# syghmon/bridges-with-reinforcement-learning

Measured on AMD Instinct MI355X. Metric: env-steps/sec (vectorised assembly_gym, tower_height=4), higher is better.
Workload: dtype f64

## Files before the change

### bridges-with-reinforcement-learning_amd/csrc/api.hip

```cpp
#include <hip/hip_runtime.h>
#include <cstdio>
#include <cstdlib>
#include <cstring>
#include <new>

#include "env_kernels.hip"
#include "ops_kernels.hip"
#include "dqn_kernels.hip"
#include "mlp_kernels.hip"
#include "conv_kernels.hip"
#include "conv_train_kernels.hip"

using namespace bridges;

static thread_local char g_err[512] = "";

static int fail_hip(hipError_t e, const char* what) {
    snprintf(g_err, sizeof(g_err), "%s: %s", what, hipGetErrorString(e));
    return BRIDGES_E_HIP;
}
static int fail_arg(const char* what) {
    snprintf(g_err, sizeof(g_err), "bad argument: %s", what);
    return BRIDGES_E_ARG;
}
// ... 172 lines not shown
    *out = env;
    return BRIDGES_OK;
}

static void free_events(bridges_env* env) {
    for (int i = 0; i < env->ev_cap; ++i) {
        (void)hipEventDestroy(env->ev_start[i]);
        (void)hipEventDestroy(env->ev_stop[i]);
    }
    delete[] env->ev_start;
    delete[] env->ev_stop;
    env->ev_start = env->ev_stop = nullptr;
    env->ev_cap = env->ev_used = 0;
}

int bridges_env_destroy(bridges_env* env) {
    if (!env) return BRIDGES_OK;
    free_events(env);
    if (env->raster_done) (void)hipEventDestroy(env->raster_done);
    (void)hipFree(env->tt_dev);
    (void)hipHostFree(env->h_total);
    delete env;
    return BRIDGES_OK;
}

int bridges_gate_create(bridges_gate** out) {
    if (!out) return fail_arg("gate_create");
    bridges_gate* g = new (std::nothrow) bridges_gate();
    if (!g) return fail_arg("oom");
    g->last = nullptr;
    *out = g;
    return BRIDGES_OK;
}

int bridges_gate_destroy(bridges_gate* gate) {
    delete gate;
    return BRIDGES_OK;
}

int bridges_env_set_gate(bridges_env* env, bridges_gate* gate) {
    if (!env) return fail_arg("set_gate");
    if (gate && !env->raster_done) HIP_TRY(hipEventCreateWithFlags(&env->raster_done, hipEventDisableTiming));
    env->gate = gate;
    return BRIDGES_OK;
}

int bridges_env_timing_begin(bridges_env* env, int32_t max_launches) {
    if (!env || max_launches <= 0 || max_launches > (1 << 16)) return fail_arg("timing_begin");
    free_events(env);
    env->ev_start = new (std::nothrow) hipEvent_t[max_launches];
    env->ev_stop = new (std::nothrow) hipEvent_t[max_launches];
    if (!env->ev_start || !env->ev_stop) {
        delete[] env->ev_start;
        delete[] env->ev_stop;
        env->ev_start = env->ev_stop = nullptr;
        return fail_arg("oom");
    }
    for (int i = 0; i < max_launches; ++i) {
        HIP_TRY(hipEventCreate(&env->ev_start[i]));
        HIP_TRY(hipEventCreate(&env->ev_stop[i]));
        env->ev_cap = i + 1;
    }
    env->ev_used = 0;
    return BRIDGES_OK;
}

int bridges_env_timing_end(bridges_env* env, double* raster_ms_total, int32_t* n_launches) {
    if (!env || !raster_ms_total || !n_launches) return fail_arg("timing_end");
    double total = 0.0;
    for (int i = 0; i < env->ev_used; ++i) {
        HIP_TRY(hipEventSynchronize(env->ev_stop[i]));
        float ms = 0.f;
        HIP_TRY(hipEventElapsedTime(&ms, env->ev_start[i], env->ev_stop[i]));
        total += ms;
    }
    *raster_ms_total = total;
    *n_launches = env->ev_used;
    free_events(env);
    return BRIDGES_OK;
}

static int refresh(bridges_env* env, hipStream_t s, int after_step) {
    const DevCtx& c = env->ctx;
    if (int rc = launch("k_scan", k_scan, dim3(1), dim3(SCAN_THREADS), 0, s, c, after_step)) return rc;
    if (int rc = launch("k_enumerate", k_enumerate, dim3(c.E), dim3(WAVE), 0, s, c)) return rc;
    const long long items_est = candidate_estimate(env) + c.E;
    long long rblocks = ceil_div(items_est, 4);
    if (rblocks > env->max_blocks) rblocks = env->max_blocks;
    const bool timed = env->ev_cap > 0 && env->ev_used < env->ev_cap;
    if (env->gate && env->gate->last) HIP_TRY(hipStreamWaitEvent(s, env->gate->last, 0));
    if (timed) HIP_TRY(hipEventRecord(env->ev_start[env->ev_used], s));
    if (!env->has_tasks) {
        if (int rc = launch("k_raster", env->max_faces <= 4 ? k_raster<4> : k_raster<MAXV>, dim3((unsigned)rblocks), dim3(256), 0, s, c))
            return rc;
    } else if (env->tasks.n_obstacles == 0) {
        if (int rc = launch("k_raster (per-env tables)", env->max_faces <= 4 ? k_raster<4, true> : k_raster<MAXV, true>,
                            dim3((unsigned)rblocks), dim3(256), 0, s, c))
            return rc;
    } else if (int rc = launch("k_raster (per-env tables and obstacles)", env->max_faces <= 4 ? k_raster<4, true, const uint64_t*> : k_raster<MAXV, true, const uint64_t*>,
                               dim3((unsigned)rblocks), dim3(256), 0, s, c, (const uint64_t*)env->tasks.env_obstacle_bits)) {
        return rc;
    }
    if (timed) { HIP_TRY(hipEventRecord(env->ev_stop[env->ev_used], s)); env->ev_used++; }
    if (env->gate) {
        HIP_TRY(hipEventRecord(env->raster_done, s));
        env->gate->last = env->raster_done;
    }
    return launch("k_select", k_select, dim3(c.E), dim3(WAVE), 0, s, c, 0);
}

static int task_features(bridges_env* env, void* stream, int mode) {
    if (env->family.family != BRIDGES_FAMILY_NONE && env->family_thr)
        return launch("k_task_features (weighted task family)", k_task_features<bridges_task_family, const uint64_t*>, dim3(env->ctx.E),
                      dim3(TASK_THREADS), 0, stream, env->ctx, env->tasks, mode, env->family, env->family_thr);
    if (env->family.family != BRIDGES_FAMILY_NONE)
        return launch("k_task_features (task family)", k_task_features<bridges_task_family>, dim3(env->ctx.E), dim3(TASK_THREADS), 0,
                      stream, env->ctx, env->tasks, mode, env->family);
    return launch("k_task_features", k_task_features<>, dim3(env->ctx.E), dim3(TASK_THREADS), 0, stream, env->ctx, env->tasks, mode);
}

int bridges_env_reset(bridges_env* env, void* stream) {
    if (!env) return fail_arg("null env");
    if (int rc = launch("k_reset", k_reset, dim3(env->ctx.E), dim3(WAVE), 0, stream, env->ctx)) return rc;
    if (env->has_tasks)
        if (int rc = task_features(env, stream, TASK_RESET)) return rc;
    return refresh(env, (hipStream_t)stream, 0);
}

int bridges_env_step(bridges_env* env, void* stream) {
    if (!env) return fail_arg("null env");
    if (!env->has_tasks) {
        if (int rc = launch("k_step", k_step<>, dim3(env->ctx.E), dim3(WAVE), 0, stream, env->ctx)) return rc;
    } else {
        if (int rc = launch("k_step (per-env targets)", k_step<const double*>, dim3(env->ctx.E), dim3(WAVE), 0, stream, env->ctx,
                            (const double*)env->tasks.env_targets))
            return rc;
        if (env->tasks.sample || env->tasks.sample_obstacles || env->family.family != BRIDGES_FAMILY_NONE)
            if (int rc = task_features(env, stream, TASK_STEP)) return rc;
    }
    return refresh(env, (hipStream_t)stream, 1);
}

int bridges_env_set_task_buffers(bridges_env* env, const bridges_task_buffers* tb) {
    if (!env) return fail_arg("null env");
    DevCtx& c = env->ctx;
    if (!tb) {
        clear_family(env);
        env->has_tasks = false;
        memset(&env->tasks, 0, sizeof(env->tasks));
        c.b.reward_map = env->fixed_reward_map;
        c.b.reward_prefix = env->fixed_reward_prefix;
        return BRIDGES_OK;
    }
    if (!tb->env_targets || !tb->target_bits || !tb->reward_map || !tb->reward_prefix || !tb->task_episode || !tb->gauss_k)
        return fail_arg("task buffers: env_targets / target_bits / reward_map / reward_prefix / task_episode / gauss_k not given");
    if (tb->n_obstacles < 0 || tb->n_obstacles > BRIDGES_MAX_OBSTACLES) return fail_arg("task buffers: n_obstacles must be 0..BRIDGES_MAX_OBSTACLES");
    if (tb->env_obstacle_bits && tb->n_obstacles == 0) return fail_arg("task buffers: env_obstacle_bits given but n_obstacles is 0");
    if (tb->n_obstacles > 0 && !tb->env_obstacle_bits) return fail_arg("task buffers: n_obstacles > 0 but env_obstacle_bits not given");
    if (tb->n_obstacles > 0 && !tb->env_obstacles) return fail_arg("task buffers: n_obstacles > 0 but env_obstacles not given");
    if (tb->n_obstacles == 0 && tb->env_obstacles) return fail_arg("task buffers: env_obstacles given but n_obstacles is 0");
    if (tb->sample_obstacles != 0 && tb->sample_obstacles != 1) return fail_arg("task buffers: sample_obstacles must be 0 or 1");
    if (tb->sample_obstacles && tb->n_obstacles == 0) return fail_arg("task buffers: sample_obstacles needs n_obstacles > 0");
    if (tb->sample_obstacles)
        for (int o = 0; o < tb->n_obstacles; ++o)
            if (!(tb->obs_x_range[o][0] <= tb->obs_x_range[o][1] && tb->obs_z_range[o][0] <= tb->obs_z_range[o][1]))
                return fail_arg("task buffers: obs_x_range / obs_z_range");
    if (c.n_targets < 1) return fail_arg("task buffers: the task has no targets");
    if (tb->target_shape < 0 || tb->target_shape >= c.n_shapes) return fail_arg("task buffers: target_shape");
// ... 1 lines not shown
    if (tb->sample && !(tb->x_range[0] <= tb->x_range[1] && tb->z_range[0] <= tb->z_range[1])) return fail_arg("task buffers: x_range / z_range");
    env->tasks = *tb;
    clear_family(env);
    env->has_tasks = true;
    c.b.reward_map = tb->reward_map;
    c.b.reward_prefix = tb->reward_prefix;
    return BRIDGES_OK;
}

int bridges_env_set_task_family(bridges_env* env, const bridges_task_family* fam) {
    if (!env) return fail_arg("null env");
    if (!fam || fam->family == BRIDGES_FAMILY_NONE) {
        clear_family(env);
        return BRIDGES_OK;
    }
    if (fam->family != BRIDGES_FAMILY_SPAN && fam->family != BRIDGES_FAMILY_TOWER) return fail_arg("task family: family must be NONE, SPAN or TOWER");
    if (!env->has_tasks) return fail_arg("task family: no task buffers attached");
    if (env->ctx.n_targets != 1) return fail_arg("task family: the task must have n_targets == 1");
    if (fam->n_hi < 1 || fam->n_hi > BRIDGES_MAX_OBSTACLES) return fail_arg("task family: n_hi must be 1..BRIDGES_MAX_OBSTACLES");
    if (fam->n_lo < 0 || fam->n_lo > fam->n_hi) return fail_arg("task family: 0 <= n_lo <= n_hi");
    if (env->tasks.n_obstacles != fam->n_hi) return fail_arg("task family: the task buffers must have n_obstacles == n_hi");
    if (!(fam->size > 0.0)) return fail_arg("task family: size must be > 0");
    if (!fam->task_class) return fail_arg("task family: task_class not given");
    env->family = *fam;
    env->family_thr = nullptr;
    return BRIDGES_OK;
}

int bridges_env_set_family_thresholds(bridges_env* env, const uint64_t* thr_dev) {
    if (!env) return fail_arg("null env");
    if (env->family.family == BRIDGES_FAMILY_NONE) return fail_arg("family thresholds: no task family set");
    env->family_thr = thr_dev;
    return BRIDGES_OK;
}

int bridges_env_load_targets(bridges_env* env, void* stream) {
    if (!env) return fail_arg("null env");
    if (!env->has_tasks) return fail_arg("bridges_env_load_targets: no task buffers attached");
    return task_features(env, stream, TASK_LOAD);
}

int bridges_env_refresh(bridges_env* env, void* stream) {
    if (!env) return fail_arg("null env");
    return refresh(env, (hipStream_t)stream, 0);
}

#define CS_TAB_SMALL 768
#define CS_COLS_SMALL 92
#define CS_TAB_LARGE 4096
int bridges_env_candidate_stability(bridges_env* env, void* stream) {
    if (!env) return fail_arg("null env");
    const DevCtx& c = env->ctx;
    if (!c.b.cand_stable || !c.b.cand_queue || !c.b.cand_counters || !c.b.cand_ws) return fail_arg("cand_stable / cand_queue / cand_counters / cand_ws not given");
    if (c.b.cand_ws_stride < (int64_t)(3 * c.K + 2) * (4 * BRIDGES_MAX_INTERFACES + 3)) return fail_arg("cand_ws_stride");
    hipStream_t s = (hipStream_t)stream;
    HIP_TRY(hipMemsetAsync(c.b.cand_counters, 0, 2 * sizeof(int32_t), s));
    long long est = candidate_estimate(env);
    if (est > env->max_blocks) est = env->max_blocks;
    if (int rc = launch("k_candidate_stability", k_candidate_stability<CS_TAB_SMALL, CS_COLS_SMALL, false>, dim3((unsigned)est),
                        dim3(WAVE), 0, s, c))
        return rc;
    const int drain = BRIDGES_CAND_WS_SLOTS;
    return launch("k_candidate_stability (queue)", k_candidate_stability<CS_TAB_LARGE, LP_MAX_COLS, true>, dim3(drain), dim3(WAVE),
                  0, s, c);
}

int bridges_env_restrict_to_stable(bridges_env* env, void* stream) {
    if (!env) return fail_arg("null env");
    if (int rc = bridges_env_candidate_stability(env, stream)) return rc;
    return launch("k_restrict_stable", k_restrict_stable, dim3(env->ctx.E), dim3(WAVE), 0, stream, env->ctx);
}

int bridges_env_rebuild_contacts(bridges_env* env, void* stream) {
    if (!env) return fail_arg("null env");
    return launch("k_rebuild_contacts", k_rebuild_contacts, dim3(env->ctx.E), dim3(WAVE), 0, stream, env->ctx);
}

int bridges_env_select_random(bridges_env* env, void* stream) {
    if (!env) return fail_arg("null env");
    return launch("k_select", k_select, dim3(env->ctx.E), dim3(WAVE), 0, stream, env->ctx, 1);
}

int bridges_env_lockstep_random(bridges_env* env, void* stream) {
    if (int rc = bridges_env_select_random(env, stream)) return rc;
    return bridges_env_step(env, stream);
}

int bridges_shapes_upload(const bridges_shape* host, int32_t n, bridges_shape** out_dev) {
    if (!host || n <= 0 || !out_dev) return fail_arg("shapes_upload");
    HIP_TRY(hipMalloc((void**)out_dev, sizeof(bridges_shape) * n));
    HIP_TRY(hipMemcpy(*out_dev, host, sizeof(bridges_shape) * n, hipMemcpyHostToDevice));
    return BRIDGES_OK;
}

int bridges_shapes_free(bridges_shape* dev) {
    if (dev) HIP_TRY(hipFree(dev));
    return BRIDGES_OK;
}

int bridges_place(const bridges_shape* shapes_dev, int32_t n, const double* frame1, const int32_t* shape_id,
                  const int32_t* face, const double* ox, const double* oy, double* pose, double* verts, void* stream) {
    if (n < 0 || !shapes_dev) return fail_arg("bridges_place");
    if (n == 0) return BRIDGES_OK;
    return launch("k_place", k_place, dim3(ceil_div(n, 256)), dim3(256), 0, stream, shapes_dev, n, frame1, shape_id, face, ox, oy,
                  pose, verts);
}

int bridges_create_block(const bridges_shape* shapes_dev, int32_t n, const double* target_verts,
                         const int32_t* target_shape, const int32_t* target_face, const int32_t* shape_id,
                         const int32_t* face, const double* ox, const double* oy, double* pose, double* verts,
                         double* target_frame_out, void* stream) {
    if (n < 0 || !shapes_dev) return fail_arg("bridges_create_block");
    if (n == 0) return BRIDGES_OK;
    return launch("k_create_block", k_create_block, dim3(ceil_div(n, 256)), dim3(256), 0, stream, shapes_dev, n, target_verts,
                  target_shape, target_face, shape_id, face, ox, oy, pose, verts, target_frame_out);
}

int bridges_pose_block(const bridges_shape* shapes_dev, int32_t n, const int32_t* shape_id, const double* pose,
                       double* verts, void* stream) {
    if (n < 0 || !shapes_dev) return fail_arg("bridges_pose_block");
    if (n == 0) return BRIDGES_OK;
    return launch("k_pose_block", k_pose_block, dim3(ceil_div(n, 256)), dim3(256), 0, stream, shapes_dev, n, shape_id, pose, verts);
}

int bridges_face_frames(const bridges_shape* shapes_dev, int32_t n, const int32_t* shape_id, const double* verts,
                        double* frames, void* stream) {
    if (n < 0 || !shapes_dev) return fail_arg("bridges_face_frames");
    if (n == 0) return BRIDGES_OK;
    return launch("k_face_frames", k_face_frames, dim3(ceil_div(n, 256)), dim3(256), 0, stream, shapes_dev, n, shape_id, verts, frames);
}

int bridges_contains_points(const bridges_shape* shapes_dev, int32_t shape_id, const double* verts, int32_t n,
                            const double* points, uint8_t* inside, void* stream) {
    if (n < 0 || !shapes_dev) return fail_arg("bridges_contains_points");
    if (n == 0) return BRIDGES_OK;
    return launch("k_contains_points", k_contains_points, dim3(ceil_div(n, 256)), dim3(256), 0, stream, shapes_dev, shape_id, verts,
                  n, points, inside);
}

int bridges_render_blocks(const bridges_shape* shapes_dev, int32_t n, const double* verts, const int32_t* shape_id,
                          const double* grid_x, int32_t W, const double* grid_y, int32_t H, uint8_t* out, void* stream) {
    if (!shapes_dev || n < 0 || W < 1 || H < 1 || !grid_x || !grid_y || !out || (n > 0 && (!verts || !shape_id)))
        return fail_arg("bridges_render_blocks");
    const int64_t px = (int64_t)W * H;
    return launch("k_render_blocks", k_render_blocks, dim3((unsigned)ceil_div(px, 256)), dim3(256), 0, stream, shapes_dev, n, verts,
                  shape_id, grid_x, W, grid_y, H, out);
}

int bridges_raster_sized(const bridges_shape* shapes_dev, int32_t n, const double* verts, const int32_t* shape_id,
                         const double* grid_x, const double* grid_y, int32_t size, uint64_t* bits, float* img,
                         void* stream) {
    if (n < 0 || !shapes_dev) return fail_arg("bridges_raster");
    if (size < 2 || size > IMG) return fail_arg("bridges_raster: image size must be 2..64");
    if (n == 0) return BRIDGES_OK;
    return launch("k_raster_generic", k_raster_generic, dim3(grid_for_waves(n)), dim3(256), 0, stream, shapes_dev, n, verts, shape_id,
                  grid_x, grid_y, (int)size, bits, img);
}

int bridges_raster(const bridges_shape* shapes_dev, int32_t n, const double* verts, const int32_t* shape_id,
                   const double* grid_x, const double* grid_y, uint64_t* bits, float* img, void* stream) {
    return bridges_raster_sized(shapes_dev, n, verts, shape_id, grid_x, grid_y, IMG, bits, img, stream);
}

int bridges_action_features(const bridges_shape* shapes_dev, int32_t n, const double* verts, const int32_t* shape_id,
                            const double* grid_x, const double* grid_y, int32_t size, double xlim0, double xlim1, double ylim0,
                            double ylim1, const uint64_t* state_bits, const uint64_t* obstacle_bits, const double* reward_prefix,
                            uint64_t* bits, float* img, uint8_t* mask, float* lin_reward, void* stream) {
    if (n < 0 || !shapes_dev || !verts || !shape_id || !grid_x || !grid_y) return fail_arg("bridges_action_features");
// ... 841 lines not shown
```

### bridges-with-reinforcement-learning_amd/csrc/env_kernels.hip

```cpp
#include "bridges_device.h"
#include "rbe_device.h"

namespace bridges {

__device__ inline void reset_env(const DevCtx& c, int e, int lane) {
    c.b.state_bits[(size_t)e * IMG + lane] = 0ull;
    if (lane < c.K) c.b.blk_occ[(size_t)e * c.K + lane] = 0;
    if (lane == 0) {
        c.b.n_blocks[e] = 0;
        c.b.n_if[e] = 0;
        c.b.targets_left[e] = (c.n_targets >= 32) ? 0xffffffffu : ((1u << c.n_targets) - 1u);
        c.b.needs_reset[e] = 0;
    }
}

__device__ inline int count_candidates(const DevCtx& c, int e, int nb, int lane) {
    int nfree = 0;
    for (int i0 = 0; i0 < nb * MAXV; i0 += WAVE) {
        int i = i0 + lane;
        bool fr = false;
        if (i < nb * MAXV) {
            int b = i / MAXV, f = i % MAXV;
            int nv = c.tt->shapes[c.b.blk_shape[(size_t)e * c.K + b]].nv;
            fr = f < nv && !((c.b.blk_occ[(size_t)e * c.K + b] >> f) & 1);
        }
        nfree += __popcll(__ballot(fr));
    }
    return c.n_groups * (c.n_ground + nfree * c.n_offsets);
}

__global__ __launch_bounds__(WAVE) void k_reset(DevCtx c) {
    int e = blockIdx.x, lane = threadIdx.x;
    reset_env(c, e, lane);
    if (lane < 8) c.b.step_flags[(size_t)e * 8 + lane] = 0;
    int nc = count_candidates(c, e, 0, lane);
    if (lane == 0) {
        c.b.reward[e] = 0.f;
        c.b.lin_reward[e] = 0.f;
        c.b.n_reached[e] = 0;
        c.b.draw_counter[e] = 0;
        c.b.n_cand[e] = nc;
    }
}

#define STEP_IF_LDS 32
#define STEP_TAB_LDS 4096
struct StepStage {
    bridges_shape shapes[8];
    double pose[MAXK * 4];
    double verts[MAXK * MAXV * 2];
    int32_t shape_id[MAXK];
    int32_t occ[MAXK];
};
struct StepKeep {
    double if_geom[STEP_IF_LDS * 8];
    int32_t if_body[STEP_IF_LDS * 2];
    double cen[MAXK * 2];
    double vol[MAXK];
};
static_assert(sizeof(StepStage) <= STEP_TAB_LDS * sizeof(double), "staging area must fit into the tableau storage");

__device__ __forceinline__ const double* step_targets() { return nullptr; }
__device__ __forceinline__ const double* step_targets(const double* p) { return p; }
template <typename... ENV_TARGETS>
__global__ __launch_bounds__(WAVE) void k_step(DevCtx c, ENV_TARGETS... env_targets_arg) {
    constexpr bool PER_ENV = sizeof...(ENV_TARGETS) == 1;
    const double* env_targets = step_targets(env_targets_arg...);
    (void)env_targets;
    __shared__ __attribute__((aligned(16))) double tab[STEP_TAB_LDS];
    __shared__ LpScratch S;
    __shared__ StepKeep Lk;
    StepStage& L = *reinterpret_cast<StepStage*>(tab);
    __builtin_amdgcn_s_setprio(3);
    const int e = blockIdx.x, lane = threadIdx.x;
    const int K = c.K;
    uint8_t* flags = c.b.step_flags + (size_t)e * 8;
    int32_t* shape_id_g = c.b.blk_shape + (size_t)e * K;
    double* pose_g = c.b.blk_pose + (size_t)e * K * 4;
    double* verts_g = c.b.blk_verts + (size_t)e * K * MAXV * 2;
    uint8_t* occ_g = c.b.blk_occ + (size_t)e * K;
    int32_t* if_body_g = c.b.if_body + (size_t)e * MAXIF * 2;
    double* if_geom_g = c.b.if_geom + (size_t)e * MAXIF * 8;
    double* ws = c.b.lp_ws + (size_t)e * c.b.lp_ws_stride;
    const WarmHdr* hdr_g = reinterpret_cast<const WarmHdr*>(ws);

    const uint8_t need_reset = c.b.needs_reset[e];
    const int a = c.b.sel_index[e];
    const int off = c.b.cand_offset[e];
    const int nb = c.b.n_blocks[e];
    const int n_if_old = c.b.n_if[e];
    uint32_t left = c.b.targets_left[e];
    const uint64_t sbits = c.b.state_bits[(size_t)e * IMG + lane];
    WarmPre W;
    W.magic = hdr_g->magic; W.n_blocks = hdr_g->n_blocks; W.n_if = hdr_g->n_if; W.stride = hdr_g->stride;
    W.half = hdr_g->half; W.m = hdr_g->m;
    W.basis_lane = hdr_g->basis[lane];
    double tgv = 0.0;
    if constexpr (PER_ENV) {
        if (lane < c.n_targets * 3) tgv = env_targets[(size_t)e * c.n_targets * 3 + lane];
    }
    {
        const double* src = reinterpret_cast<const double*>(c.tt->shapes);
        double* dst = reinterpret_cast<double*>(L.shapes);
        const int nd = c.n_shapes * (int)(sizeof(bridges_shape) / 8);
        for (int i = lane; i < nd; i += WAVE) dst[i] = src[i];
        for (int i = lane; i < nb * 4; i += WAVE) L.pose[i] = pose_g[i];
        for (int i = lane; i < nb * MAXV * 2; i += WAVE) L.verts[i] = verts_g[i];
        if (lane < K) { L.shape_id[lane] = shape_id_g[lane]; L.occ[lane] = occ_g[lane]; }
        const int n0 = n_if_old < STEP_IF_LDS ? n_if_old : STEP_IF_LDS;
        for (int i = lane; i < n0 * 8; i += WAVE) Lk.if_geom[i] = if_geom_g[i];
        for (int i = lane; i < n0 * 2; i += WAVE) Lk.if_body[i] = if_body_g[i];
    }

    if (need_reset) {
        reset_env(c, e, lane);
        if (lane < 8) flags[lane] = 0;
        if (lane == 0) {
            c.b.reward[e] = 0.f;
            c.b.lin_reward[e] = 0.f;
            c.b.n_reached[e] = 0;
        }
        if (lane == 0) c.b.n_cand[e] = c.n_groups * c.n_ground;
        return;
    }

    const size_t ci = (size_t)off + a;
    const int dsc = lane < 4 ? c.b.cand_desc[ci * 4 + lane] : 0;
    const double cpose = lane < 4 ? c.b.cand_pose[ci * 4 + lane] : 0.0;
    const double cvert = lane < MAXV * 2 ? c.b.cand_verts[ci * MAXV * 2 + lane] : 0.0;
    const uint64_t cbits = c.b.cand_bits[ci * IMG + lane];
    const float base = c.b.cand_lin[ci];
    warm_prefetch(W, ws, nb, n_if_old, lane);
    const int tb = __builtin_amdgcn_readlane(dsc, 0), tf = __builtin_amdgcn_readlane(dsc, 1);
    const int sh = __builtin_amdgcn_readlane(dsc, 2), fc = __builtin_amdgcn_readlane(dsc, 3);

    if (lane < 4) { L.pose[nb * 4 + lane] = cpose; pose_g[nb * 4 + lane] = cpose; }
    if (lane < MAXV * 2) { L.verts[nb * MAXV * 2 + lane] = cvert; verts_g[nb * MAXV * 2 + lane] = cvert; }
    c.b.state_bits[(size_t)e * IMG + lane] = sbits | cbits;
    __syncthreads();
    if (lane == 0) {
        L.shape_id[nb] = sh;
        shape_id_g[nb] = sh;
        L.occ[nb] = (int32_t)(1u << fc);
        occ_g[nb] = (uint8_t)(1u << fc);
        if (tb >= 0) {
            L.occ[tb] |= (int32_t)(1u << tf);
            occ_g[tb] = (uint8_t)L.occ[tb];
        }
        c.b.n_blocks[e] = nb + 1;
    }
    __syncthreads();
    const bridges_shape* shapes = L.shapes;
    const bridges_shape& shn = shapes[sh];
    int nf = 0;
    if (lane <= nb) {
        const bridges_shape& sb = shapes[L.shape_id[lane]];
        double rgx, rgz;
        rot2(sb.gx, sb.gz, L.pose[4 * lane + 2], L.pose[4 * lane + 3], rgx, rgz);
        Lk.cen[2 * lane] = L.pose[4 * lane] + rgx;
        Lk.cen[2 * lane + 1] = L.pose[4 * lane + 1] + rgz;
        Lk.vol[lane] = sb.volume;
        nf = sb.nv - __popc((uint32_t)L.occ[lane] & ((1u << sb.nv) - 1u));
    }

    double vx = 0.0, vz = 0.0;
    const int nvn = shn.nv;
    bool hasv = lane < nvn;
    if (hasv) { vx = L.verts[nb * MAXV * 2 + 2 * lane]; vz = L.verts[nb * MAXV * 2 + 2 * lane + 1]; }
    double x0 = wave_min_d(hasv ? vx : 1e300), x1 = wave_max_d(hasv ? vx : -1e300);
    double z0 = wave_min_d(hasv ? vz : 1e300), z1 = wave_max_d(hasv ? vz : -1e300);
    {
        double cx = (x0 + x1) * 0.5, cz = (z0 + z1) * 0.5, hx = (x1 - x0) * 0.5, hz = (z1 - z0) * 0.5;
        double hy = shn.depth * 0.5;
        bool skip = false;
        for (int t = 0; t < c.n_targets; ++t) {
            if (!((left >> t) & 1u)) continue;
            if (skip) { skip = false; continue; }
            bool in;
            if constexpr (PER_ENV) {
                const double tx = readlane_d(tgv, 3 * t), ty = readlane_d(tgv, 3 * t + 1), tz = readlane_d(tgv, 3 * t + 2);
                in = fabs(tx - cx) < hx + 1e-6 && fabs(ty) < hy + 1e-6 && fabs(tz - cz) < hz + 1e-6;
            } else {
                in = fabs(c.targets[t][0] - cx) < hx + 1e-6 && fabs(c.targets[t][1]) < hy + 1e-6 &&
                     fabs(c.targets[t][2] - cz) < hz + 1e-6;
            }
            if (in) { left &= ~(1u << t); skip = true; }
        }
    }
    const int n_reached = c.n_targets - __popc(left);

    int n_if = n_if_old;
    bool overflow = false;
    {
        const double* nverts = L.verts + nb * MAXV * 2;
        const int totalp = (1 + nb * MAXV) * MAXV;
// ... 97 lines not shown
    if (t == 0) carry_s = 0;
    __syncthreads();
    unsigned long long acc[8] = {0, 0, 0, 0, 0, 0, 0, 0};
    for (int base0 = 0; base0 < c.E; base0 += SCAN_THREADS * SCAN_BATCH) {
        int v[SCAN_BATCH], nbk[SCAN_BATCH], nval[SCAN_BATCH];
        uint64_t fl8[SCAN_BATCH];
#pragma unroll
        for (int u = 0; u < SCAN_BATCH; ++u) {
            const int i = base0 + u * SCAN_THREADS + t;
            const bool in = i < c.E;
            v[u] = in ? c.b.n_cand[i] : 0;
            nbk[u] = in ? c.b.n_blocks[i] : 0;
            nval[u] = (in && after_step) ? c.b.n_valid[i] : 0;
            fl8[u] = (in && after_step) ? *reinterpret_cast<const uint64_t*>(c.b.step_flags + (size_t)i * 8) : 0ull;
        }
#pragma unroll
        for (int u = 0; u < SCAN_BATCH; ++u) {
            const int base = base0 + u * SCAN_THREADS;
            if (base >= c.E) break;
            const int i = base + t;
            if (i < c.E) {
                if (v[u] > c.a_max) {
                    v[u] = c.a_max;
                    c.b.n_cand[i] = c.a_max;
                    c.b.step_flags[(size_t)i * 8 + F_LP_ERROR] |= 8;
                    acc[7] += 1;
                }
                acc[0] += (unsigned long long)nbk[u];
                if (after_step) {
                    const unsigned valid = (unsigned)(fl8[u] >> (8 * F_VALID)) & 0xffu;
                    const unsigned lperr = (unsigned)(fl8[u] >> (8 * F_LP_ERROR)) & 0xffu;
                    acc[1] += valid ? 1 : 0;
                    acc[2] += valid ? 0 : 1;
                    acc[3] += (lperr & 1) ? 1 : 0;
                    acc[4] += (lperr & 2) ? 1 : 0;
                    acc[5] += (unsigned long long)nval[u];
                    acc[6] += (lperr & 4) ? 1 : 0;
                }
            }
            int incl = v[u];
#pragma unroll
            for (int o = 1; o < WAVE; o <<= 1) {
                int up = __shfl_up(incl, o, WAVE);
                if (lane >= o) incl += up;
            }
            if (lane == WAVE - 1) wave_tot[wv] = incl;
            __syncthreads();
            int wbase = 0;
            for (int k = 0; k < wv; ++k) wbase += wave_tot[k];
            const int carry = carry_s;
            if (i < c.E) c.b.cand_offset[i] = carry + wbase + incl - v[u];
            __syncthreads();
            if (t == SCAN_THREADS - 1) carry_s = carry + wbase + incl;
            __syncthreads();
        }
    }
#pragma unroll
    for (int k = 0; k < 8; ++k) {
        unsigned long long x = acc[k];
#pragma unroll
        for (int o = 32; o > 0; o >>= 1) x += __shfl_xor(x, o, WAVE);
        if (lane == 0) red[wv][k] = x;
    }
    __syncthreads();
    if (t == 0) {
        unsigned long long tot[8] = {0, 0, 0, 0, 0, 0, 0, 0};
        for (int w = 0; w < SCAN_WAVES; ++w)
            for (int k = 0; k < 8; ++k) tot[k] += red[w][k];
        c.b.cand_offset[c.E] = carry_s;
        if (c.h_total) *c.h_total = carry_s;
        c.b.stats[ST_SUM_CAND] += (uint64_t)carry_s;
        c.b.stats[ST_SUM_BLOCKS] += tot[0];
        c.b.stats[ST_ENV_STEPS] += tot[1];
        c.b.stats[ST_RESET_ONLY] += tot[2];
        c.b.stats[ST_LP_ERRORS] += tot[3];
        c.b.stats[ST_IF_OVERFLOW] += tot[4];
        c.b.stats[ST_SUM_VALID] += tot[5];
        c.b.stats[ST_WARM_RESOLVED] += tot[6];
        c.b.stats[ST_CAND_OVERFLOW] += tot[7];
        c.b.stats[ST_LOCKSTEPS] += 1;
    }
}

__global__ __launch_bounds__(WAVE) void k_enumerate(DevCtx c) {
    __shared__ uint8_t free_b[MAXK * MAXV], free_f[MAXK * MAXV];
    __shared__ bridges_shape sh_l[8];
    __shared__ double verts_l[MAXK * MAXV * 2];
    __shared__ int32_t shape_l[MAXK], occ_l[MAXK];
    __shared__ double xg_l[32], offs_l[8];
    __builtin_amdgcn_s_setprio(3);
    const int e = blockIdx.x, lane = threadIdx.x;
    const int K = c.K;
    if (lane < 32) xg_l[lane] = c.tt->x_ground[lane];
    if (lane < 8) offs_l[lane] = c.tt->offsets[lane];
    const int nb = c.b.n_blocks[e];
    const int ncand = c.b.n_cand[e];
    const size_t off = (size_t)c.b.cand_offset[e];
    {
        const double* src = reinterpret_cast<const double*>(c.tt->shapes);
        double* dst = reinterpret_cast<double*>(sh_l);
        const int nd = c.n_shapes * (int)(sizeof(bridges_shape) / 8);
        for (int i = lane; i < nd; i += WAVE) dst[i] = src[i];
        const double* vg = c.b.blk_verts + (size_t)e * K * MAXV * 2;
        for (int i = lane; i < nb * MAXV * 2; i += WAVE) verts_l[i] = vg[i];
        if (lane < K) { shape_l[lane] = c.b.blk_shape[(size_t)e * K + lane]; occ_l[lane] = c.b.blk_occ[(size_t)e * K + lane]; }
    }
    __syncthreads();
    const bridges_shape* shapes = sh_l;
    const int32_t* shape_id = shape_l;
    const double* verts = verts_l;
    int nfree = 0;
    for (int i0 = 0; i0 < nb * MAXV; i0 += WAVE) {
        int i = i0 + lane;
        bool fr = false;
        int b = i / MAXV, f = i % MAXV;
        if (i < nb * MAXV) {
            int nv = shapes[shape_id[b]].nv;
            fr = f < nv && !((occ_l[b] >> f) & 1);
        }
        uint64_t bal = __ballot(fr);
        if (fr) {
            int idx = nfree + __popcll(bal & ((1ull << lane) - 1ull));
            free_b[idx] = (uint8_t)b;
            free_f[idx] = (uint8_t)f;
        }
        nfree += __popcll(bal);
    }
    __syncthreads();
    const int gsize = c.n_ground + nfree * c.n_offsets;
    for (int a = lane; a < ncand; a += WAVE) {
        int grp = a / gsize, slot = a % gsize;
        int sh = c.group_shape[grp], fc = c.group_face[grp];
        int tb = -1, tf = 0;
        double ox;
        Frame2 f1;
        if (slot < c.n_ground) {
            ox = xg_l[slot];
            f1.cx = 0.0; f1.cz = 0.0; f1.tx = 1.0; f1.tz = 0.0; f1.nx = 0.0; f1.nz = 1.0;
        } else {
            int k = (slot - c.n_ground) / c.n_offsets;
            ox = offs_l[(slot - c.n_ground) % c.n_offsets];
            tb = free_b[k]; tf = free_f[k];
            const bridges_shape& st = shapes[shape_id[tb]];
            const double* v = verts + (size_t)tb * MAXV * 2;
            f1 = edge_frame(v[2 * st.fa[tf]], v[2 * st.fa[tf] + 1], v[2 * st.fb[tf]], v[2 * st.fb[tf] + 1]);
        }
        const bridges_shape& sn = shapes[sh];
        double px, pz, cs, sn_;
        align_place(f1, sn.fcx[fc], sn.fcz[fc], sn.fnx[fc], sn.fnz[fc], ox, 0.0, px, pz, cs, sn_);
        const size_t ci = off + a;
        bool inb = true;
        const double eps = 1e-6;
        double wx[MAXV], wz[MAXV];
#pragma unroll
        for (int i = 0; i < MAXV; ++i) {
            wx[i] = 0.0; wz[i] = 0.0;
            if (i < sn.nv) {
                double rx, rz;
                rot2(sn.vx[i], sn.vz[i], cs, sn_, rx, rz);
                wx[i] = px + rx; wz[i] = pz + rz;
                if (wx[i] < c.xlim0 - eps || wx[i] > c.xlim1 + eps || wz[i] < c.ylim0 - eps || wz[i] > c.ylim1 + eps) inb = false;
                if (wz[i] < -eps) inb = false;
            }
            c.b.cand_verts[ci * MAXV * 2 + 2 * i] = wx[i];
            c.b.cand_verts[ci * MAXV * 2 + 2 * i + 1] = wz[i];
        }
        {
#define PICK6(v, k) ((k) == 5 ? v[5] : (k) == 4 ? v[4] : (k) == 3 ? v[3] : (k) == 2 ? v[2] : (k) == 1 ? v[1] : v[0])
#pragma unroll
            for (int f = 0; f < MAXV; ++f) {
                double o0 = 0.0, o1 = 0.0, o2 = 0.0, o3 = 0.0;
                if (f < sn.nv) {
                    const int ia = sn.fa[f], ib = sn.fb[f];
                    const double ax = PICK6(wx, ia), az = PICK6(wz, ia), bx = PICK6(wx, ib), bz = PICK6(wz, ib);
                    Frame2 fr = edge_frame(ax, az, bx, bz);
                    o0 = fr.cx; o1 = fr.cz; o2 = fr.nx; o3 = fr.nz;
                }
                double2* dst = reinterpret_cast<double2*>(c.b.cand_frames + (ci * MAXV + f) * 4);
                dst[0] = make_double2(o0, o1);
                dst[1] = make_double2(o2, o3);
            }
#undef PICK6
            c.b.cand_rows[ci * 2 + 0] = (sn.nv << 16) | ((inb ? 1 : 0) << 24);
            c.b.cand_rows[ci * 2 + 1] = e;
        }
        c.b.cand_pose[ci * 4 + 0] = px; c.b.cand_pose[ci * 4 + 1] = pz;
        c.b.cand_pose[ci * 4 + 2] = cs; c.b.cand_pose[ci * 4 + 3] = sn_;
        c.b.cand_desc[ci * 4 + 0] = tb; c.b.cand_desc[ci * 4 + 1] = tf;
        c.b.cand_desc[ci * 4 + 2] = sh; c.b.cand_desc[ci * 4 + 3] = fc;
        c.b.cand_ox[ci] = ox;
        c.b.cand_inb[ci] = inb;
        c.b.cand_env[ci] = e;
    }
}

__device__ __forceinline__ void write_f32_image(float* img, uint64_t rowbits, int lane, int32_t* nz = nullptr) {
    const int sub = lane >> 4, col4 = (lane & 15) * 4;
    const uint64_t nonzero_rows = __ballot(rowbits != 0ull);
    if (nz) {
        uint64_t t = nonzero_rows | (nonzero_rows >> 1);
        t = (t | (t >> 2)) & 0x1111111111111111ull;
        uint32_t now = 0u;
#pragma unroll
        for (int g = 0; g < IMG / 4; ++g) now |= (uint32_t)((t >> (4 * g)) & 1ull) << g;
        uint32_t need = (uint32_t)__builtin_amdgcn_readfirstlane(*nz) | now;
        if (lane == 0) *nz = (int32_t)now;
        while (need) {
            const int g = __builtin_ctz(need);
            need &= need - 1u;
            uint32_t nib = 0u;
            if ((now >> g) & 1u) {
                uint64_t m = shfl_u64(rowbits, 4 * g + sub);
                nib = (uint32_t)(m >> col4) & 0xFu;
            }
            float4 v;
            v.x = (nib & 1u) ? 1.f : 0.f;
            v.y = (nib & 2u) ? 1.f : 0.f;
            v.z = (nib & 4u) ? 1.f : 0.f;
            v.w = (nib & 8u) ? 1.f : 0.f;
            *reinterpret_cast<float4*>(img + (size_t)(4 * g + sub) * IMG + col4) = v;
        }
        return;
    }
#pragma unroll
    for (int r0 = 0; r0 < IMG; r0 += 4) {
        uint32_t nib = 0u;
        if ((nonzero_rows >> r0) & 0xFull) {
            uint64_t m = shfl_u64(rowbits, r0 + sub);
            nib = (uint32_t)(m >> col4) & 0xFu;
        }
        float4 v;
        v.x = (nib & 1u) ? 1.f : 0.f;
        v.y = (nib & 2u) ? 1.f : 0.f;
        v.z = (nib & 4u) ? 1.f : 0.f;
        v.w = (nib & 8u) ? 1.f : 0.f;
        *reinterpret_cast<float4*>(img + (size_t)(r0 + sub) * IMG + col4) = v;
    }
}

__device__ __forceinline__ uint64_t low_mask64(int n) { return n >= 64 ? ~0ull : ((1ull << n) - 1ull); }

template <int NF, int F0 = 0>
__device__ __forceinline__ uint64_t raster_rows(double fr0, double fr1, double fr2, double fr3, int n_img, double X, double Y,
                                                int lane) {
    int alo[NF], ahi[NF], pos[NF];
    double t[NF];
    bool rev[NF];
#pragma unroll
    for (int f = 0; f < NF; ++f) {
        const double cxf = readlane_d(fr0, F0 + f), czf = readlane_d(fr1, F0 + f), nxf = readlane_d(fr2, F0 + f), nzf = readlane_d(fr3, F0 + f);
        const double a = (X - cxf) * nxf;
        t[f] = -((Y - czf) * nzf);
        alo[f] = __double2loint(a);
        ahi[f] = __double2hiint(a);
        rev[f] = nxf < 0.0;
        pos[f] = 0;
    }
#define RASTER_PROBE(S_, INC_)                                                                                          \
    _Pragma("unroll") for (int f = 0; f < NF; ++f) {                                                                    \
        const int j = pos[f] + (S_);                                                                                    \
        const int src = rev[f] ? 63 - j : j;                                                                            \
        const double av = __hiloint2double(__shfl(ahi[f], src, WAVE), __shfl(alo[f], src, WAVE));                       \
        if (av <= t[f]) pos[f] += (INC_);                                                                               \
    }
    RASTER_PROBE(31, 32) RASTER_PROBE(15, 16) RASTER_PROBE(7, 8) RASTER_PROBE(3, 4) RASTER_PROBE(1, 2) RASTER_PROBE(0, 1)
    RASTER_PROBE(0, 1)
#undef RASTER_PROBE
    uint64_t bits = low_mask64(n_img);
#pragma unroll
    for (int f = 0; f < NF; ++f) {
        const uint64_t run = low_mask64(pos[f]);
        bits &= rev[f] ? (pos[f] ? ~low_mask64(64 - pos[f]) : 0ull) : run;
    }
    return lane < n_img ? bits : 0ull;
}
// ... 586 lines not shown
```

Before: 4.806 million.

## Fuse scan into enumerate and random selection into step kernel

Measured after the change: 4.750 million. 0.988x the previous value.

```diff
diff --git a/bridges-with-reinforcement-learning_amd/csrc/api.hip b/bridges-with-reinforcement-learning_amd/csrc/api.hip
--- a/bridges-with-reinforcement-learning_amd/csrc/api.hip
+++ b/bridges-with-reinforcement-learning_amd/csrc/api.hip
@@ -278,8 +278,12 @@
 
 static int refresh(bridges_env* env, hipStream_t s, int after_step) {
     const DevCtx& c = env->ctx;
-    if (int rc = launch("k_scan", k_scan, dim3(1), dim3(SCAN_THREADS), 0, s, c, after_step)) return rc;
-    if (int rc = launch("k_enumerate", k_enumerate, dim3(c.E), dim3(WAVE), 0, s, c)) return rc;
+    if (c.E <= ENUM_SCAN_MAX_E) {
+        if (int rc = launch("k_enumerate", k_enumerate<true>, dim3(c.E), dim3(WAVE), 0, s, c, after_step)) return rc;
+    } else {
+        if (int rc = launch("k_scan", k_scan, dim3(1), dim3(SCAN_THREADS), 0, s, c, after_step)) return rc;
+        if (int rc = launch("k_enumerate (after k_scan)", k_enumerate<false>, dim3(c.E), dim3(WAVE), 0, s, c, after_step)) return rc;
+    }
     const long long items_est = candidate_estimate(env) + c.E;
     long long rblocks = ceil_div(items_est, 4);
     if (rblocks > env->max_blocks) rblocks = env->max_blocks;
@@ -447,8 +451,17 @@
 }
 
 int bridges_env_lockstep_random(bridges_env* env, void* stream) {
-    if (int rc = bridges_env_select_random(env, stream)) return rc;
-    return bridges_env_step(env, stream);
+    if (!env) return fail_arg("null env");
+    if (!env->has_tasks) {
+        if (int rc = launch("k_step (draw)", k_step<StepDraw>, dim3(env->ctx.E), dim3(WAVE), 0, stream, env->ctx, StepDraw{})) return rc;
+    } else {
+        if (int rc = launch("k_step (draw, per-env targets)", k_step<const double*, StepDraw>, dim3(env->ctx.E), dim3(WAVE), 0, stream,
+                            env->ctx, (const double*)env->tasks.env_targets, StepDraw{}))
+            return rc;
+        if (env->tasks.sample || env->tasks.sample_obstacles || env->family.family != BRIDGES_FAMILY_NONE)
+            if (int rc = task_features(env, stream, TASK_STEP)) return rc;
+    }
+    return refresh(env, (hipStream_t)stream, 1);
 }
 
 int bridges_shapes_upload(const bridges_shape* host, int32_t n, bridges_shape** out_dev) {
diff --git a/bridges-with-reinforcement-learning_amd/csrc/env_kernels.hip b/bridges-with-reinforcement-learning_amd/csrc/env_kernels.hip
--- a/bridges-with-reinforcement-learning_amd/csrc/env_kernels.hip
+++ b/bridges-with-reinforcement-learning_amd/csrc/env_kernels.hip
@@ -60,12 +60,78 @@
 };
 static_assert(sizeof(StepStage) <= STEP_TAB_LDS * sizeof(double), "staging area must fit into the tableau storage");
 
+struct StepDraw {};
 __device__ __forceinline__ const double* step_targets() { return nullptr; }
 __device__ __forceinline__ const double* step_targets(const double* p) { return p; }
-template <typename... ENV_TARGETS>
-__global__ __launch_bounds__(WAVE) void k_step(DevCtx c, ENV_TARGETS... env_targets_arg) {
-    constexpr bool PER_ENV = sizeof...(ENV_TARGETS) == 1;
-    const double* env_targets = step_targets(env_targets_arg...);
+__device__ __forceinline__ const double* step_targets(StepDraw) { return nullptr; }
+__device__ __forceinline__ const double* step_targets(const double* p, StepDraw) { return p; }
+template <typename T, typename... A>
+constexpr bool step_has_arg = (std::is_same<T, A>::value || ... || false);
+#define STEP_DRAW_ROUNDS 4
+
+__device__ __forceinline__ int step_draw(const DevCtx& c, int e, int lane, size_t off, int nc) {
+    const uint8_t* mask = c.b.cand_mask + off;
+    const uint64_t ctr = c.b.draw_counter[e];
+    uint8_t m[STEP_DRAW_ROUNDS];
+#pragma unroll
+    for (int u = 0; u < STEP_DRAW_ROUNDS; ++u) {
+        const int a = u * WAVE + lane;
+        m[u] = a < nc ? mask[a] : (uint8_t)0;
+    }
+    uint64_t bal[STEP_DRAW_ROUNDS];
+    int nvalid = 0;
+#pragma unroll
+    for (int u = 0; u < STEP_DRAW_ROUNDS; ++u) {
+        bal[u] = __ballot(m[u] != 0);
+        nvalid += __popcll(bal[u]);
+    }
+    for (int a0 = STEP_DRAW_ROUNDS * WAVE; a0 < nc; a0 += WAVE) {
+        const int a = a0 + lane;
+        nvalid += __popcll(__ballot(a < nc && mask[a]));
+    }
+    int sel = 0;
+    if (nvalid > 0) {
+        const uint64_t r = splitmix64(splitmix64(((c.seed & 0xFFFFFFFFull) << 32) | (uint32_t)(c.env_id_base + e)) ^ ctr);
+        const int rank = (int)(r % (uint64_t)nvalid);
+        int seen = 0;
+        bool found = false;
+#pragma unroll
+        for (int u = 0; u < STEP_DRAW_ROUNDS; ++u) {
+            const int cnt = __popcll(bal[u]);
+            if (!found && rank < seen + cnt) {
+                uint64_t b = bal[u];
+                const int want = rank - seen;
+                for (int k = 0; k < want; ++k) b &= b - 1;
+                sel = u * WAVE + (__ffsll((long long)b) - 1);
+                found = true;
+            }
+            seen += cnt;
+        }
+        for (int a0 = STEP_DRAW_ROUNDS * WAVE; !found && a0 < nc; a0 += WAVE) {
+            const int a = a0 + lane;
+            uint64_t b = __ballot(a < nc && mask[a]);
+            const int cnt = __popcll(b);
+            if (rank < seen + cnt) {
+                const int want = rank - seen;
+                for (int k = 0; k < want; ++k) b &= b - 1;
+                sel = a0 + (__ffsll((long long)b) - 1);
+                found = true;
+            }
+            seen += cnt;
+        }
+    }
+    if (lane == 0) {
+        c.b.sel_index[e] = sel;
+        if (nvalid > 0) c.b.draw_counter[e] = ctr + 1;
+    }
+    return __builtin_amdgcn_readfirstlane(sel);
+}
+
+template <typename... STEP_ARGS>
+__global__ __launch_bounds__(WAVE) void k_step(DevCtx c, STEP_ARGS... step_args) {
+    constexpr bool PER_ENV = step_has_arg<const double*, STEP_ARGS...>;
+    constexpr bool DRAW = step_has_arg<StepDraw, STEP_ARGS...>;
+    const double* env_targets = step_targets(step_args...);
     (void)env_targets;
     __shared__ __attribute__((aligned(16))) double tab[STEP_TAB_LDS];
     __shared__ LpScratch S;
@@ -85,7 +151,8 @@
     const WarmHdr* hdr_g = reinterpret_cast<const WarmHdr*>(ws);
 
     const uint8_t need_reset = c.b.needs_reset[e];
-    const int a = c.b.sel_index[e];
+    int a = 0;
+    if constexpr (!DRAW) a = c.b.sel_index[e];
     const int off = c.b.cand_offset[e];
     const int nb = c.b.n_blocks[e];
     const int n_if_old = c.b.n_if[e];
@@ -111,6 +178,7 @@
         for (int i = lane; i < n0 * 8; i += WAVE) Lk.if_geom[i] = if_geom_g[i];
         for (int i = lane; i < n0 * 2; i += WAVE) Lk.if_body[i] = if_body_g[i];
     }
+    if constexpr (DRAW) a = step_draw(c, e, lane, (size_t)off, c.b.n_cand[e]);
 
     if (need_reset) {
         reset_env(c, e, lane);
@@ -374,7 +442,80 @@
     }
 }
 
-__global__ __launch_bounds__(WAVE) void k_enumerate(DevCtx c) {
+#define ENUM_SCAN_MAX_E 8192
+#define ENUM_SCAN_BATCH 32
+__device__ __forceinline__ unsigned long long wave_sum_u64(unsigned long long x) {
+#pragma unroll
+    for (int o = 32; o > 0; o >>= 1) x += __shfl_xor(x, o, WAVE);
+    return x;
+}
+template <typename LOAD>
+__device__ __forceinline__ unsigned long long enum_sum(int n, int lane, LOAD load) {
+    unsigned long long sum = 0;
+    for (int j0 = 0; j0 < n; j0 += WAVE * ENUM_SCAN_BATCH) {
+        decltype(load(0)) v[ENUM_SCAN_BATCH];
+#pragma unroll
+        for (int u = 0; u < ENUM_SCAN_BATCH; ++u) {
+            const int j = j0 + u * WAVE + lane;
+            v[u] = j < n ? load(j) : 0;
+        }
+#pragma unroll
+        for (int u = 0; u < ENUM_SCAN_BATCH; ++u) sum += (unsigned long long)v[u];
+    }
+    return wave_sum_u64(sum);
+}
+__device__ __forceinline__ int enum_offset(const DevCtx& c, int n, int lane) {
+    int sum = 0;
+    for (int j0 = 0; j0 < n; j0 += WAVE * ENUM_SCAN_BATCH) {
+        int v[ENUM_SCAN_BATCH];
+#pragma unroll
+        for (int u = 0; u < ENUM_SCAN_BATCH; ++u) {
+            const int j = j0 + u * WAVE + lane;
+            v[u] = j < n ? c.b.n_cand[j] : 0;
+        }
+#pragma unroll
+        for (int u = 0; u < ENUM_SCAN_BATCH; ++u) sum += v[u] < c.a_max ? v[u] : c.a_max;
+    }
+#pragma unroll
+    for (int o = 32; o > 0; o >>= 1) sum += __shfl_xor(sum, o, WAVE);
+    return sum;
+}
+#define ENUM_STAT_PARTS 4
+__device__ __forceinline__ unsigned long long enum_stats_sum(const DevCtx& c, int lane, int part) {
+    if (part == 0) return enum_sum(c.E, lane, [&](int j) { const int v = c.b.n_cand[j]; return v < c.a_max ? v : c.a_max; });
+    if (part == 1) return enum_sum(c.E, lane, [&](int j) { return c.b.n_blocks[j]; });
+    if (part == 2) return enum_sum(c.E, lane, [&](int j) { return c.b.n_valid[j]; });
+    static_assert(ENUM_SCAN_MAX_E < (1 << 16), "the packed counters hold 16 bits each");
+    return enum_sum(c.E, lane, [&](int j) {
+        const uint64_t fl8 = *reinterpret_cast<const uint64_t*>(c.b.step_flags + (size_t)j * 8);
+        const unsigned valid = (unsigned)(fl8 >> (8 * F_VALID)) & 0xffu, lperr = (unsigned)(fl8 >> (8 * F_LP_ERROR)) & 0xffu;
+        return (unsigned long long)(valid ? 1 : 0) | (unsigned long long)(lperr & 1) << 16 |
+               (unsigned long long)((lperr >> 1) & 1) << 32 | (unsigned long long)((lperr >> 2) & 1) << 48;
+    });
+}
+__device__ __forceinline__ void enum_stats_store(const DevCtx& c, int part, unsigned long long sum) {
+    if (part == 0) {
+        c.b.stats[ST_SUM_CAND] += sum;
+        c.b.stats[ST_LOCKSTEPS] += 1;
+    } else if (part == 1) {
+        c.b.stats[ST_SUM_BLOCKS] += sum;
+    } else if (part == 2) {
+        c.b.stats[ST_SUM_VALID] += sum;
+    } else {
+        const unsigned long long steps = sum & 0xffffu;
+        c.b.stats[ST_ENV_STEPS] += steps;
+        c.b.stats[ST_RESET_ONLY] += (unsigned long long)c.E - steps;
+        c.b.stats[ST_LP_ERRORS] += (sum >> 16) & 0xffffu;
+        c.b.stats[ST_IF_OVERFLOW] += (sum >> 32) & 0xffffu;
+        c.b.stats[ST_WARM_RESOLVED] += (sum >> 48) & 0xffffu;
+    }
+}
+__device__ __forceinline__ bool enum_stats_mine(const DevCtx& c, int e, int after_step, int part) {
+    return (part == e || (part > e && e == c.E - 1)) && (after_step || part < 2);
+}
+
+template <bool SCAN>
+__global__ __launch_bounds__(WAVE) void k_enumerate(DevCtx c, int after_step) {
     __shared__ uint8_t free_b[MAXK * MAXV], free_f[MAXK * MAXV];
     __shared__ bridges_shape sh_l[8];
     __shared__ double verts_l[MAXK * MAXV * 2];
@@ -386,8 +527,20 @@
     if (lane < 32) xg_l[lane] = c.tt->x_ground[lane];
     if (lane < 8) offs_l[lane] = c.tt->offsets[lane];
     const int nb = c.b.n_blocks[e];
-    const int ncand = c.b.n_cand[e];
-    const size_t off = (size_t)c.b.cand_offset[e];
+    int ncand = c.b.n_cand[e];
+    size_t off;
+    bool cut = false;
+    unsigned long long stat[ENUM_STAT_PARTS] = {0, 0, 0, 0};
+    if constexpr (SCAN) {
+        off = (size_t)enum_offset(c, e, lane);
+        cut = ncand > c.a_max;
+        if (cut) ncand = c.a_max;
+#pragma unroll
+        for (int p = 0; p < ENUM_STAT_PARTS; ++p)
+            if (enum_stats_mine(c, e, after_step, p)) stat[p] = enum_stats_sum(c, lane, p);
+    } else {
+        off = (size_t)c.b.cand_offset[e];
+    }
     {
         const double* src = reinterpret_cast<const double*>(c.tt->shapes);
         double* dst = reinterpret_cast<double*>(sh_l);
@@ -483,6 +636,23 @@
         c.b.cand_ox[ci] = ox;
         c.b.cand_inb[ci] = inb;
         c.b.cand_env[ci] = e;
+    }
+    if constexpr (SCAN) {
+        if (lane == 0) {
+            if (cut) {
+                c.b.n_cand[e] = c.a_max;
+                c.b.step_flags[(size_t)e * 8 + F_LP_ERROR] |= 8;
+                atomicAdd(reinterpret_cast<unsigned long long*>(c.b.stats + ST_CAND_OVERFLOW), 1ull);
+            }
+            c.b.cand_offset[e] = (int)off;
+            if (e == c.E - 1) {
+                c.b.cand_offset[c.E] = (int)off + ncand;
+                if (c.h_total) *c.h_total = (int)off + ncand;
+            }
+#pragma unroll
+            for (int p = 0; p < ENUM_STAT_PARTS; ++p)
+                if (enum_stats_mine(c, e, after_step, p)) enum_stats_store(c, p, stat[p]);
+        }
     }
 }
 
```
